# arcosoph/nanowakeword

Hardware: AMD Instinct MI355X
Metric: clips/sec (1 s @16 kHz PCM->logits) (higher is better)
Workload: dtype f32; 1 GPU; cnn head on (101,64) log-mel, batch=4096/GPU, 1 s 16 kHz mono int16 clips, 64-mel 25 ms/10 ms center frontend, fused STFT+mel HIP kernel, fp32; clips_per_gpu=4096, n_samples=16000, parallelism=batch-split x1

## Files before the change

### nanowakeword_amd/csrc/layers.h

```cpp
#pragma once
#include <hip/hip_runtime.h>

#include <map>
#include <mutex>
#include <utility>
inline hipError_t nww_allow_lds(const void* func, size_t bytes) {
    if (bytes <= 64 * 1024) return hipSuccess;
    static std::mutex mu;
    static std::map<std::pair<int, const void*>, size_t> done;
    int dev = 0;
    hipError_t e = hipGetDevice(&dev);
    if (e != hipSuccess) return e;
    std::lock_guard<std::mutex> lk(mu);
    size_t& cur = done[std::make_pair(dev, func)];
    if (bytes > cur) {
        e = hipFuncSetAttribute(func, hipFuncAttributeMaxDynamicSharedMemorySize, (int)bytes);
        if (e != hipSuccess) return e;
        cur = bytes;
    }
    return hipSuccess;
}

__device__ __forceinline__ float nww_silu(float v) {
    return v * __builtin_amdgcn_rcpf(1.0f + __builtin_amdgcn_exp2f(v * -1.4426950408889634f));
// ... 31 lines not shown
    int h2 = 0; float a_scale = 1.0f, c_scale = 1.0f, a_clamp = 0.0f;
    int a_blocked = 0;
    const float* A2 = nullptr; int lda2 = 0; const float* W2 = nullptr; int K2 = 0;
    const float* alpha2 = nullptr; const float* beta2 = nullptr;
};
size_t gemm_x3_weight_bytes(int N, int K);
hipError_t launch_split_weights_x3(const float* W, void* out, int N, int K, hipStream_t s);
hipError_t launch_split_weights_h2(const float* W, void* out, int N, int K, float scale, hipStream_t s);
bool gemm_x3_usable(const GemmArgs& g);
bool gemm_writes_partials(const GemmArgs& g);
hipError_t launch_gemm_x3(const GemmArgs& g, hipStream_t s);
int gemm_recommended_splitk(long long M, int N, int K, int cu_count);
hipError_t launch_gemm(const GemmArgs& g, hipStream_t s);

struct Conv3Args {
    const float* in; const float* w; const float* bias; const float* alpha; const float* beta;
    float* out; int B, Cin, Cout, H, W; int act; int pool;
    int nhwc_out = 0;
};
hipError_t launch_conv3x3(const Conv3Args& a, hipStream_t s);

hipError_t launch_dwconv3x3_nhwc(const float* in, const float* wt, float* d_out, float* xs_out, int B, int C, int H,
                                 int W, int sh, int sw, hipStream_t s, int act16 = 0, float out_mul = 1.0f);
hipError_t launch_layernorm_parts(const float* parts, int nparts, size_t part_stride, const float* in_bias, float* y, const float* w,
                                  const float* b, int R, int D, int act, hipStream_t s);
hipError_t launch_layernorm(const float* x, float* y, const float* w, const float* b, int R, int D, int act,
                            hipStream_t s);
hipError_t launch_mean_mid(const float* in, float* out, int B, int L, int D, hipStream_t s, int act16 = 0, float unscale = 1.0f);
hipError_t launch_ln_mean(const float* x, float* out, const float* w, const float* b, int B, int L, int D, hipStream_t s);
hipError_t launch_avgpool(const float* in, float* out, int BC, int H, int W, int kh, int kw, int sh, int sw, int oh,
                          int ow, hipStream_t s);
hipError_t launch_unary(const float* x, float* y, size_t n, int act, hipStream_t s);
hipError_t launch_scale_add_pe(float* x, const float* pe, int B, int T, int D, float scale, hipStream_t s);
hipError_t launch_glu(const float* in, float* out, int R, int D, hipStream_t s);
hipError_t launch_dwconv1d_bn_swish(const float* x, const float* w , const float* bias, const float* alpha,
                                    const float* beta, float* y, int B, int T, int D, int K, hipStream_t s);
hipError_t launch_mha_core(const float* qkv, float* out, int B, int T, int D, int n_head, hipStream_t s);
bool mha_mfma_supported(int T, int D, int n_head);
hipError_t launch_mha_mfma(const float* qkv, float* out, int B, int T, int D, int n_head, int cus, hipStream_t s, int head_major = 0);
bool mha_head_dim_supported(int head_dim);
bool mha_h2_supported(int T, int D, int n_head);
hipError_t launch_mha_h2(const float* qkv, float* out, int B, int T, int D, int n_head, int cus, hipStream_t s, int head_major = 0, int exact_sub = 0);
hipError_t launch_crnn_seq(const float* in, float* out, int B, int C, int H, int W, hipStream_t s);
struct GruArgs {
    const float* xg; const float* w_hh; const float* b_hh;
    float* seq_out; int ld_seq; float* last_out; int ld_last; int col_off;
    int B, T, H, reverse, steps;
    int products = 0;
    float w_scale = 1.0f;
    const float* xg2 = nullptr; size_t xg2_bstride = 0; const float* b_hh2 = nullptr; int col_off2 = 0;
    int ldw = 0;
    const float* x_in = nullptr; const float* w_ih = nullptr; const float* b_ih = nullptr;
    int fin = 0; float x_scale = 1.0f, x_clamp = 0.0f, wi_scale = 1.0f;
    const void* w_packed = nullptr;
    int cu_count = 256;
    int dbg = 0;
};
size_t rnn_wide_weight_bytes(int gates, int H);
hipError_t launch_rnn_pad_weights(const float* w_hh, float* out, int gates, int H, hipStream_t s);
hipError_t launch_gru(const GruArgs& a, hipStream_t s);
hipError_t launch_transpose3x3(const float* w, float* out, int nfilters, hipStream_t s);
hipError_t launch_transpose_planes(const float* in, float* out, int B, int R, int C, hipStream_t s);
bool rnn_x3_usable(const GruArgs& a);
hipError_t launch_rnn_x3(const GruArgs& a, int gates, hipStream_t s);
bool rnn_stream_usable(const GruArgs& a);
size_t rnn_stream_packed_bytes(int gates, int H);
hipError_t launch_rnn_stream_pack(const float* w_hh, void* packed, int gates, int H, float w_scale, hipStream_t s);
hipError_t launch_rnn_stream(const GruArgs& a, int gates, hipStream_t s);
hipError_t launch_lstm(const GruArgs& a, hipStream_t s);

struct TailArgs {
    const float* x; int Kin;
    const float *We, *be; int E;
    const float *W0, *b0, *w3, *b3;
    float *emb, *logits, *probs;
    int B, act;
    const float* parts = nullptr; int nparts = 0; size_t part_stride = 0;
    const float *in_bias = nullptr, *in_alpha = nullptr, *in_beta = nullptr; int in_act = 0;
    unsigned int* done_flag = nullptr; unsigned int done_seq = 0;
    const float *ln0_w = nullptr, *ln0_b = nullptr;
    int n_mid = 0;
    const float *mid_W[4] = {nullptr, nullptr, nullptr, nullptr}, *mid_b[4] = {nullptr, nullptr, nullptr, nullptr};
    const float *mid_lnw[4] = {nullptr, nullptr, nullptr, nullptr}, *mid_lnb[4] = {nullptr, nullptr, nullptr, nullptr};
};
bool tail_supported(int Kin, int E);
hipError_t launch_classifier_tail(const TailArgs& a, hipStream_t s);
```

### nanowakeword_amd/csrc/layers.hip

```cpp
#include <hip/hip_runtime.h>
#include <stdint.h>
#include <stdlib.h>
#include "layers.h"
#include "split_h2.h"

typedef float f32x16 __attribute__((ext_vector_type(16)));
typedef float f32x4 __attribute__((ext_vector_type(4)));

__device__ __forceinline__ float act_apply(float v, int act) {
    switch (act) {
        case ACT_RELU: return fmaxf(v, 0.0f);
        case ACT_GELU: return nww_gelu(v);
        case ACT_SILU: return v / (1.0f + expf(-v));
        case ACT_SIGMOID: return 1.0f / (1.0f + expf(-v));
        default: return v;
    }
}

template <int ACT>
__device__ __forceinline__ float act_ct(float v) {
    if (ACT == ACT_RELU) return fmaxf(v, 0.0f);
    if (ACT == ACT_GELU) return nww_gelu(v);
    if (ACT == ACT_SILU) return v / (1.0f + expf(-v));
    if (ACT == ACT_SIGMOID) return 1.0f / (1.0f + expf(-v));
// ... 1607 lines not shown
                    const size_t o = (size_t)(b0 + cc) * Kin + k;
                    float acc = 0.0f;
                    for (int z0 = 0; z0 < a.nparts; z0 += 8) {
                        float pv[8];
#pragma unroll
                        for (int j = 0; j < 8; ++j) pv[j] = z0 + j < a.nparts ? a.parts[(size_t)(z0 + j) * a.part_stride + o] : 0.0f;
#pragma unroll
                        for (int j = 0; j < 8; ++j)
                            if (z0 + j < a.nparts) acc = (z0 + j == 0) ? pv[j] : acc + pv[j];
                    }
                    v = acc + (a.in_bias ? a.in_bias[k] : 0.0f);
                    if (a.in_alpha) v = v * a.in_alpha[k] + a.in_beta[k];
                    v = act_apply(v, a.in_act);
                } else {
                    v = a.x[(size_t)(b0 + cc) * Kin + k];
                }
            }
            xs[cc * ldx + k] = v;
        }
        __syncthreads();
        if (a.ln0_w) {
            tile_ln(xs, xs, a.ln0_w, a.ln0_b);
            __syncthreads();
            for (int m = 0; m < a.n_mid; ++m) {
                const float* Wm = a.mid_W[m];
                const bool vm = (Kin & 3) == 0 && ((reinterpret_cast<uintptr_t>(Wm) & 15) == 0);
                for (int e0 = g; e0 < Kin; e0 += 4 * NG) {
                    const int e1 = min(e0 + NG, Kin - 1), e2 = min(e0 + 2 * NG, Kin - 1), e3 = min(e0 + 3 * NG, Kin - 1);
                    float acc[4];
                    tail_dot4(xs + c * ldx, Wm + (size_t)e0 * Kin, Wm + (size_t)e1 * Kin, Wm + (size_t)e2 * Kin, Wm + (size_t)e3 * Kin, Kin, vm, acc);
                    const int eo[4] = {e0, e0 + NG, e0 + 2 * NG, e0 + 3 * NG};
#pragma unroll
                    for (int r = 0; r < 4; ++r)
                        if (eo[r] < Kin) ys[c * ldx + eo[r]] = acc[r] + a.mid_b[m][eo[r]];
                }
                __syncthreads();
                tile_ln(ys, xs, a.mid_lnw[m], a.mid_lnb[m]);
                __syncthreads();
            }
        }
        for (int e0 = g; e0 < E; e0 += 4 * NG) {
            const int e1 = min(e0 + NG, E - 1), e2 = min(e0 + 2 * NG, E - 1), e3 = min(e0 + 3 * NG, E - 1);
            float acc[4];
            tail_dot4(xs + c * ldx, a.We + (size_t)e0 * Kin, a.We + (size_t)e1 * Kin, a.We + (size_t)e2 * Kin, a.We + (size_t)e3 * Kin, Kin, vx, acc);
            const int es_[4] = {e0, e0 + NG, e0 + 2 * NG, e0 + 3 * NG};
#pragma unroll
            for (int r = 0; r < 4; ++r)
                if (es_[r] < E) {
                    const float v = acc[r] + (a.be ? a.be[es_[r]] : 0.0f);
                    es[c * lde + es_[r]] = v;
                    if (b0 + c < a.B) a.emb[(size_t)(b0 + c) * E + es_[r]] = v;
                }
        }
        __syncthreads();
        for (int j0 = g; j0 < Hd; j0 += 4 * NG) {
            const int j1 = min(j0 + NG, Hd - 1), j2 = min(j0 + 2 * NG, Hd - 1), j3 = min(j0 + 3 * NG, Hd - 1);
            float acc[4];
            tail_dot4(es + c * lde, a.W0 + (size_t)j0 * E, a.W0 + (size_t)j1 * E, a.W0 + (size_t)j2 * E, a.W0 + (size_t)j3 * E, E, ve, acc);
            const int js[4] = {j0, j0 + NG, j0 + 2 * NG, j0 + 3 * NG};
#pragma unroll
            for (int r = 0; r < 4; ++r)
                if (js[r] < Hd) hs[c * ldh + js[r]] = act_ct<ACT>(acc[r] + a.b0[js[r]]);
        }
        __syncthreads();
        if (tid < CT && b0 + tid < a.B) {
            const float* hr = hs + tid * ldh;
            float acc = 0.0f;
            for (int j = 0; j < Hd; ++j) acc = fmaf(hr[j], a.w3[j], acc);
            const float l = acc + a.b3[0];
            a.logits[b0 + tid] = l;
            if (a.probs) a.probs[b0 + tid] = 1.0f / (1.0f + expf(-l));
            if (a.done_flag) __threadfence_system();
        }
        __syncthreads();
    }
    if (a.done_flag && gridDim.x == 1 && tid == 0) {
        __threadfence_system();
        __hip_atomic_store(a.done_flag, a.done_seq, __ATOMIC_RELEASE, __HIP_MEMORY_SCOPE_SYSTEM);
    }
}

bool tail_supported(int Kin, int E) { return Kin >= 1 && Kin <= 512 && E >= 2 && E <= 256 && (E % 2) == 0; }

hipError_t launch_classifier_tail(const TailArgs& a, hipStream_t s) {
    if (!tail_supported(a.Kin, a.E)) return hipErrorInvalidValue;
    if (a.ln0_w && (a.Kin > 256 || a.n_mid < 0 || a.n_mid > 4)) return hipErrorInvalidValue;
    const size_t lds = (size_t)16 * ((a.ln0_w ? 2 : 1) * (((a.Kin + 3) & ~3) + 4) + (((a.E + 3) & ~3) + 4) + (a.E / 2 + 1)) * sizeof(float);
    static const int ct4_max = 1024;
    const bool small = a.B <= 4 || (a.B > 16 && a.B <= ct4_max);
    const int ct = small ? 4 : 16;
    int grid = (a.B + ct - 1) / ct;
    if (grid > 1024) grid = 1024;
    if (grid < 1) grid = 1;
    if (small) {
#define TAIL_CALL(A) hipLaunchKernelGGL((classifier_tail_kernel<A, 4>), dim3(grid), dim3(256), lds, s, a)
        NWW_DISPATCH_ACT(a.act, TAIL_CALL)
#undef TAIL_CALL
    } else {
#define TAIL_CALL(A) hipLaunchKernelGGL((classifier_tail_kernel<A, 16>), dim3(grid), dim3(256), lds, s, a)
        NWW_DISPATCH_ACT(a.act, TAIL_CALL)
#undef TAIL_CALL
    }
    return hipGetLastError();
}
```

### nanowakeword_amd/csrc/nww_plan.hip

```cpp
#include "nww_internal.h"
#include "bc_chain.h"

const Knobs& nww_knobs() {
    static const Knobs k = [] {
        auto env = [](const char* name, int d) { const char* e = getenv(name); return e ? atoi(e) : d; };
        Knobs r;
        r.trunk = env("NWW_TRUNK", 1); r.conv_mfma = env("NWW_CONV_MFMA", 1); r.conv3_x3 = env("NWW_CONV3_X3", 1);
        r.gemm_x3 = env("NWW_GEMM_X3", 1); r.lin_x3 = env("NWW_LIN_X3", 1); r.ffn_fused = env("NWW_FFN_FUSED", 1);
        r.attn_fused = env("NWW_ATTN_FUSED", 1); r.mha_mfma = env("NWW_MHA_MFMA", 1); r.bc_front = env("NWW_BC_FRONT", 1);
        r.bc_chain = env("NWW_BC_CHAIN", 1); r.tail = env("NWW_TAIL", 1); r.stream_inc = env("NWW_STREAM_INC", 3);
        r.f16_range_log2 = env("NWW_F16_RANGE_LOG2", 16);
        return r;
    }();
    return k;
}

namespace {
using Shape = std::vector<int64_t>;
struct SpecBuilder {
    std::vector<std::string>& keys;
    std::map<std::string, HostTensor>& t;
    void add(const std::string& k, Shape s) { keys.push_back(k); t[k].shape = std::move(s); }
    void lin(const std::string& p, int out, int in) { add(p + ".weight", {out, in}); add(p + ".bias", {out}); }
    void ln(const std::string& p, int d) { add(p + ".weight", {d}); add(p + ".bias", {d}); }
// ... 139 lines not shown
    const float* W(const std::string& k) const {
        auto it = h->tensors.find(k);
        return it == h->tensors.end() || !it->second.loaded ? nullptr : h->d_weights + it->second.dev_off;
    }
    void need(int buf, size_t floats_per_clip) {
        if (h->buf_per_clip[buf] < floats_per_clip) h->buf_per_clip[buf] = floats_per_clip;
    }
    void add(const std::string& name, std::function<hipError_t(Run&)> fn) { h->plan.push_back({name, std::move(fn)}); }
    void pop_last() { if (!h->plan.empty()) h->plan.pop_back(); }
    std::string tail_name; int tail_in = 99, tail_K = 0; const float *tail_W = nullptr, *tail_b = nullptr;
    struct DnnBody { bool on = false; const float *ln0_w = nullptr, *ln0_b = nullptr; int n_mid = 0; const float* mid[4][4] = {}; } dnn;
};

std::vector<float> f16_fetch(nww_handle* h, const float* d, size_t n) {
    std::vector<float> v(n, 0.0f);
    if (d && n) {
        (void)hipStreamSynchronize(h->own_stream);
        if (hipMemcpy(v.data(), d, n * sizeof(float), hipMemcpyDeviceToHost) != hipSuccess) v.assign(n, INFINITY);
    }
    return v;
}
double f16_pow2_floor(double x) { int e; (void)std::frexp(x, &e); return std::ldexp(1.0, e - 1); }
float f16_scale(double bound) {
    if (!(bound > 1e-30)) bound = 1e-30;
    if (!(bound < 1e30)) return 0.0f;
    double s = f16_pow2_floor(65504.0 / (bound * 1.02));
    if (s > 1099511627776.0) s = 1099511627776.0;
    return (float)s;
}
float f16_wscale(const std::vector<float>& w) {
    double m = 0;
    for (float x : w) m = std::fmax(m, std::fabs((double)x));
    return f16_scale(m * 2.0);
}
double f16_layer_bound(const std::vector<float>& w, int Cout, int K, const std::vector<float>& b, bool has_b,
                       const std::vector<float>& al, const std::vector<float>& be, bool has_bn, double in_bound) {
    double worst = 0;
    for (int c = 0; c < Cout; ++c) {
        double t = 0;
        for (int k = 0; k < K; ++k) t += std::fabs((double)w[(size_t)c * K + k]);
        t = t * in_bound + (has_b ? std::fabs((double)b[c]) : 0.0);
        if (has_bn) t = t * std::fabs((double)al[c]) + std::fabs((double)be[c]);
        worst = std::fmax(worst, t);
    }
    return worst;
}
double f16_ln_bound(nww_handle* h, const float* w, const float* b, int D) {
    const auto hw = f16_fetch(h, w, D), hb = f16_fetch(h, b, D);
    double bound = 0.0;
    for (int k = 0; k < D; ++k) bound = std::fmax(bound, std::sqrt((double)D) * std::fabs((double)hw[k]) + std::fabs((double)hb[k]));
    return bound;
}
float f16_mean_scale(double bound) {
    const float s = bound < 1e30 ? (float)f16_pow2_floor(68719476736.0 / std::fmax(bound, 1e-30)) : 0.0f;
    return s > 0.0f && std::isfinite(s) ? s : 0.0f;
}

inline double f16_range_factor() {
    return std::ldexp(1.0, nww_knobs().f16_range_log2);
}
struct F16Range {
    double bound = 0.0, typ = 0.0;
    bool ok() const { return bound > 0.0 && typ > 0.0 && bound <= typ * f16_range_factor(); }
};
const F16Range F16_FEATURES{NWW_F16_FEATURE_BOUND, 32.0};
double f16_layer_typ(const std::vector<float>& w, int Cout, int K, const std::vector<float>& al, bool has_bn, double typ_in) {
    double acc = 0;
    for (int c = 0; c < Cout; ++c) {
        double q = 0;
        for (int k = 0; k < K; ++k) q += (double)w[(size_t)c * K + k] * (double)w[(size_t)c * K + k];
        acc += std::sqrt(q) * (has_bn ? std::fabs((double)al[c]) : 1.0);
    }
    return acc / (Cout > 0 ? Cout : 1) * typ_in;
}

inline const float* src(Run& r, int id) { return id == -1 ? r.x : id == -2 ? r.emb : id == -3 ? r.hid : r.buf[id]; }
inline float* dst(Run& r, int id) { return id == -2 ? r.emb : id == -3 ? r.hid : id == -4 ? r.logits : r.buf[id]; }

void add_gemm(PlanCtx& p, const std::string& name, int in_id, int out_id, int rows_per_clip, int N, int K,
              const float* W, const float* bias, int act, const float* alpha = nullptr, const float* beta = nullptr,
              int res_id = 99, float rscale = 1.f, bool* a_blocked_inout = nullptr, bool feeds_tail = false, bool feeds_ln = false,
              F16Range a_range = F16Range{}, bool a_bound_assumed = false) {
    const double a_bound = a_range.ok() ? a_range.bound : 0.0;
    if (out_id >= 0) p.need(out_id, (size_t)rows_per_clip * N);
    const int x3_mode = nww_knobs().gemm_x3;
    const bool small_square = N <= 160 && K > 64 && K <= 160;
    const bool use_x3 = p.h->conv_products != 0 &&
                        (x3_mode == 2 ? (N >= 32 && K >= 32)
                         : x3_mode == 3 ? (K >= 4096 && N >= 64 && N <= 256)
                         : (x3_mode == 1 && N >= 64 && K >= 32 && !small_square));
    const void* wx3 = nullptr;
    float h2_as = 0.0f, h2_ws = 0.0f;
    if (use_x3 && p.h->f16 && a_bound > 0.0) {
        h2_as = f16_scale(a_bound);
        if (h2_as > 0.0f) h2_ws = f16_wscale(f16_fetch(p.h, W, (size_t)N * K));
    }
    const bool h2_req = h2_as > 0.0f && h2_ws > 0.0f;
    if (use_x3) {
        const X3Key key{W, h2_req ? 1 : 0, h2_req ? h2_ws : 0.0f};
        auto it = p.h->x3_weights.find(key);
        if (it == p.h->x3_weights.end()) {
            void* d = nullptr;
            if (hipMalloc(&d, gemm_x3_weight_bytes(N, K)) == hipSuccess &&
                (h2_req ? launch_split_weights_h2(W, d, N, K, h2_ws, p.h->own_stream) : launch_split_weights_x3(W, d, N, K, p.h->own_stream)) == hipSuccess)
                it = p.h->x3_weights.emplace(key, d).first;
            else if (d) (void)hipFree(d);
        }
        if (it != p.h->x3_weights.end()) wx3 = it->second;
    }
    const bool h2 = h2_req && wx3 != nullptr;
    if (h2 && a_bound_assumed && in_id == -1) p.h->clamps_features = true;
    const int a_blocked = (a_blocked_inout && *a_blocked_inout && wx3 && K % 32 == 0 && rows_per_clip == 1) ? K / 32 : 0;
    if (a_blocked_inout) *a_blocked_inout = a_blocked != 0;
    if (K >= 2048 && (size_t)16 * rows_per_clip * N > p.h->splitk_per_clip) p.h->splitk_per_clip = (size_t)16 * rows_per_clip * N;
    p.add("gemm:" + name + (h2 && wx3 ? " [f16x3]" : ""), [=](Run& r) {
        GemmArgs g;
        g.A = src(r, in_id); g.lda = K; g.W = W; g.C = dst(r, out_id); g.ldc = N;
        g.M = r.B * rows_per_clip; g.N = N; g.K = K; g.bias = bias; g.alpha = alpha; g.beta = beta; g.act = act;
        g.res = res_id == 99 ? nullptr : src(r, res_id); g.ldres = N; g.rscale = rscale;
        g.Wx3 = wx3;
        if (h2) { g.h2 = 1; g.a_scale = h2_as; g.c_scale = 1.0f / (h2_as * h2_ws); g.a_clamp = a_bound_assumed ? (float)a_bound : 0.0f; }
        g.a_blocked = a_blocked;
        g.splitk = gemm_recommended_splitk(g.M, N, K, r.cu_count);
        if (wx3 && x3_mode != 2 && K >= 2048) { g.splitk = K >= 8192 ? K / 800 : K / 512; if (g.splitk > 16) g.splitk = 16; if (g.splitk < 1) g.splitk = 1; }
        g.splitk_ws = r.splitk_ws;
        if (g.splitk > 1 && (size_t)g.splitk * g.M * N > r.splitk_floats) g.splitk = 1;
        r.deferred.active = false;
        const bool partials = g.splitk > 1 && g.splitk_ws && gemm_writes_partials(g);
        if (feeds_tail && g.M <= 8 && partials && !g.res) {
            g.defer_reduce = true;
            r.deferred.active = true; r.deferred.out_id = out_id; r.deferred.parts = g.splitk; r.deferred.stride = (size_t)g.M * N;
            r.deferred.bias = bias; r.deferred.alpha = alpha; r.deferred.beta = beta; r.deferred.act = act;
        }
        if (feeds_ln && partials && !g.res && !alpha && act == ACT_NONE && N <= 256) {
            g.defer_reduce = true;
            r.deferred.active = true; r.deferred.out_id = out_id; r.deferred.parts = g.splitk; r.deferred.stride = (size_t)g.M * N;
            r.deferred.bias = bias; r.deferred.alpha = nullptr; r.deferred.beta = nullptr; r.deferred.act = ACT_NONE;
        }
        return launch_gemm(g, r.stream);
    });
}

bool add_lin_x3(PlanCtx& p, const std::string& name, int in_id, int out_id, int rows_per_clip, int N, int K, const float* W,
                const float* bias, int epi, int res_id = 99, float rscale = 1.f, const float* ln_w = nullptr,
                const float* ln_b = nullptr, int qkv_T = 0, int qkv_dh = 0, const float* res_tab = nullptr) {
    if (!nww_knobs().lin_x3 || p.h->conv_products != 6 || !lin_x3_supported(K, N, true)) return false;
    const int parts = epi == 2 ? 2 : 1;
    float ws = 0.0f;
    if (p.h->f16) ws = f16_wscale(f16_fetch(p.h, W, (size_t)parts * N * K));
    const bool h2 = ws > 0.0f;
    if (!lin_x3_supported(K, N, h2)) return false;
    const int terms = h2 ? 2 : 3;
    void* packed = nullptr;
    if (hipMalloc(&packed, lin_x3_packed_bytes(K, N, parts, terms)) != hipSuccess) return false;
    if (launch_lin_x3_pack(W, bias, packed, K, N, parts, N, p.h->own_stream, terms, h2 ? ws : 1.0f) != hipSuccess) { (void)hipFree(packed); return false; }
    p.h->packed_weights.push_back(packed);
    p.need(out_id, (size_t)rows_per_clip * N);
    const float w_un = h2 ? 1.0f / ws : 1.0f;
    p.add("lin_x3:" + name + (h2 ? " [f16x3]" : ""), [=](Run& r) {
        LinArgs a;
        a.x = src(r, in_id); a.ldx = K; a.out = dst(r, out_id); a.ldc = N;
        a.res = res_tab ? res_tab : res_id == 99 ? nullptr : src(r, res_id); a.ldres = N; a.rscale = rscale;
        a.ln_w = ln_w; a.ln_b = ln_b; a.packed = static_cast<const unsigned char*>(packed);
        a.M = r.B * rows_per_clip; a.N = N; a.qkv_T = qkv_T; a.qkv_dh = qkv_dh;
        a.h2 = h2 ? 1 : 0; a.w_un = w_un;
        return launch_lin_x3(a, K, epi, ln_w != nullptr, r.stream);
    });
    return true;
}

void add_linear(PlanCtx& p, const std::string& name, int in_id, int out_id, int rows_per_clip, int N, int K, const float* W,
                const float* bias, int res_id = 99, float rscale = 1.f) {
    if (!add_lin_x3(p, name, in_id, out_id, rows_per_clip, N, K, W, bias, res_id == 99 ? 0 : 1, res_id, rscale))
        add_gemm(p, name, in_id, out_id, rows_per_clip, N, K, W, bias, ACT_NONE, nullptr, nullptr, res_id, rscale);
}

void set_tail(PlanCtx& p, const std::string& name, int in_id, int K, const float* W, const float* b) {
    p.tail_name = name; p.tail_in = in_id; p.tail_K = K; p.tail_W = W; p.tail_b = b;
}

void add_conv(PlanCtx& p, const std::string& name, int in_id, int out_id, int Cin, int Cout, int H, int W,
              const float* w, const float* bias, const float* alpha, const float* beta, int act, int pool, int nhwc_out = 0) {
    const int Ho = pool ? H / 2 : H, Wo = pool ? W / 2 : W;
    p.need(out_id, (size_t)Cout * Ho * Wo);
    p.add("conv3x3:" + name, [=](Run& r) {
        Conv3Args a{src(r, in_id), w, bias, alpha, beta, dst(r, out_id), r.B, Cin, Cout, H, W, act, pool};
        a.nhwc_out = nhwc_out;
        return launch_conv3x3(a, r.stream);
    });
}

static int trunk_fits(int C1, int H, int W) { int per_cu = 0; return trunk_pick_strips(C1, H, W, &per_cu); }
bool add_trunk(PlanCtx& p, const std::string& name, int in_id, int out_id, int C1, int C2, int H, int W,
               const float* w1, const float* b1, const float* al1, const float* be1, const float* w2,
               const float* b2, const float* al2, const float* be2, int act, const bool* out_blocked = nullptr,
               F16Range in_range = F16Range{}, F16Range* out_range = nullptr) {
    if (out_range) *out_range = F16Range{};
    const double in_bound = in_range.ok() ? in_range.bound : 0.0;
    if (!nww_knobs().trunk || C1 != 16 || C2 != 32 || H < 4 || W < 4 || trunk_fits(C1, H, W) == 0) return false;
    p.need(out_id, (size_t)C2 * (H / 4) * (W / 4));
    const int max_grid = p.h->cu_count;
    const int x3 = p.h->conv_products;
    if ((x3 == 6 || x3 == 9) && trunk_b_pick_strips(H, W) > 0) {
        void* packed = nullptr;
        if (hipMalloc(&packed, trunk_b_packed_bytes()) != hipSuccess) return false;
        float f_in = 0.0f, f_s1 = 0.0f, f_w1 = 0.0f, f_w2 = 0.0f;
        double bound2 = 0.0, typ2 = 0.0;
        if (p.h->f16 && x3 == 6 && in_bound > 0.0 && (act == ACT_RELU || act == ACT_GELU || act == ACT_SILU)) {
            const auto hw1 = f16_fetch(p.h, w1, (size_t)C1 * 9), hw2 = f16_fetch(p.h, w2, (size_t)C2 * C1 * 9);
            const auto hb1 = f16_fetch(p.h, b1, C1), hb2 = f16_fetch(p.h, b2, C2);
            const auto ha1 = f16_fetch(p.h, al1, C1), he1 = f16_fetch(p.h, be1, C1), ha2 = f16_fetch(p.h, al2, C2), he2 = f16_fetch(p.h, be2, C2);
            const double bound1 = f16_layer_bound(hw1, C1, 9, hb1, b1 != nullptr, ha1, he1, al1 != nullptr, in_bound);
// ... 970 lines not shown
    set_tail(p, "output_proj", t1, D, p.W("model.output_proj.weight"), p.W("model.output_proj.bias"));
    return NWW_OK;
}

int plan_tcn(PlanCtx& p) {
    const nww_config& c = p.h->cfg;
    const int T = c.in_rows, F = c.in_cols;
    const int k = c.layer_dim, nl = c.n_crnn_channels;
    const int* ch = c.crnn_channels;
    const int last = 5;
    p.need(last, (size_t)ch[nl - 1]);
    auto key = [](int i, const char* part) { return "model.tcn_blocks." + std::to_string(i) + "." + part; };
    bool fused = false;
    if (p.h->f16 && p.h->conv_products == 6) {
        TcnArgs a;
        a.T = T; a.F = F; a.L = nl; a.k = k;
        for (int i = 0; i < nl; ++i) a.ch[i] = ch[i];
        std::vector<void*> packs;
        bool ok = tcn_x3_plan(a);
        int cin = F;
        for (int i = 0; ok && i < nl; ++i) {
            auto pack = [&](const char* part, int ci, int taps, TcnConv& cv) {
                const float* w = p.W(key(i, (std::string(part) + ".weight").c_str()));
                const float ws = f16_wscale(f16_fetch(p.h, w, (size_t)ch[i] * ci * taps));
                void* d = nullptr;
                if (!(ws > 0.0f) || hipMalloc(&d, tcn_x3_packed_bytes(ci, ch[i], taps)) != hipSuccess) return false;
                packs.push_back(d);
                if (launch_tcn_x3_pack(w, d, ci, ch[i], taps, ws, p.h->own_stream) != hipSuccess) return false;
                cv.packed = static_cast<const unsigned char*>(d);
                cv.bias = p.W(key(i, (std::string(part) + ".bias").c_str()));
                cv.w_un = 1.0f / ws;
                return true;
            };
            ok = pack("conv1", cin, k, a.c1[i]) && pack("conv2", ch[i], k, a.c2[i]) && (cin == ch[i] || pack("downsample", cin, 1, a.ds[i]));
            cin = ch[i];
        }
        if (ok) {
            for (void* d : packs) p.h->packed_weights.push_back(d);
            p.add("tcn_x3:" + std::to_string(nl) + " blocks, last " + std::to_string(a.S) + " steps of " + std::to_string(T) + " [f16x3]",
                  [=](Run& r) {
                      TcnArgs g = a;
                      g.x = r.x; g.out = r.buf[last]; g.B = r.B;
                      return launch_tcn_x3(g, r.stream);
                  });
            fused = true;
        } else {
            for (void* d : packs) (void)hipFree(d);
        }
    }
    if (!fused) {
        const int col = 0, hid = 1, rsd = 4;
        int in = -1, cin = F;
        for (int i = 0; i < nl; ++i) {
            const int co = ch[i], dil = 1 << i, out = i % 2 == 0 ? 2 : 3;
            const std::string q = "model.tcn_blocks." + std::to_string(i);
            p.need(col, (size_t)T * k * (cin > co ? cin : co));
            p.add("im2col:" + q + ".conv1", [=](Run& r) { return launch_tcn_im2col(src(r, in), r.buf[col], r.B, T, cin, k, dil, r.stream); });
            add_gemm(p, q + ".conv1+relu", col, hid, T, co, cin * k, p.W(key(i, "conv1.weight")), p.W(key(i, "conv1.bias")), ACT_RELU);
            p.add("im2col:" + q + ".conv2", [=](Run& r) { return launch_tcn_im2col(r.buf[hid], r.buf[col], r.B, T, co, k, dil, r.stream); });
            int res = in;
            if (cin != co) {
                add_gemm(p, q + ".downsample", in, rsd, T, co, cin, p.W(key(i, "downsample.weight")), p.W(key(i, "downsample.bias")), ACT_NONE);
                res = rsd;
            }
            add_gemm(p, q + ".conv2+relu+res", col, out, T, co, co * k, p.W(key(i, "conv2.weight")), p.W(key(i, "conv2.bias")), ACT_RELU,
                     nullptr, nullptr, res, 1.0f);
            p.add("unary:relu " + q, [=](Run& r) { return launch_unary(r.buf[out], r.buf[out], (size_t)r.B * T * co, ACT_RELU, r.stream); });
            in = out; cin = co;
        }
        const int fin = in, C = cin;
        p.add("last_row:tcn_out[:, :, T - 1]", [=](Run& r) { return launch_tcn_last_row(r.buf[fin], r.buf[last], r.B, T, C, r.stream); });
    }
    set_tail(p, "fc", last, ch[nl - 1], p.W("model.fc.weight"), p.W("model.fc.bias"));
    return NWW_OK;
}

void plan_tail(PlanCtx& p) {
    const int E = p.h->cfg.embedding_dim, act = p.h->cfg.activation;
    if (nww_knobs().tail && tail_supported(p.tail_K, E)) {
        const float *We = p.tail_W, *be = p.tail_b, *W0 = p.W("classifier.0.weight"), *b0 = p.W("classifier.0.bias"),
                    *w3 = p.W("classifier.3.weight"), *b3 = p.W("classifier.3.bias");
        const int tin = p.tail_in, tK = p.tail_K;
        const PlanCtx::DnnBody dnn = p.dnn;
        p.add("tail:" + p.tail_name + "+classifier", [=](Run& r) {
            TailArgs t{src(r, tin), tK, We, be, E, W0, b0, w3, b3, r.emb, r.logits, r.probs, r.B, act};
            if (dnn.on) {
                t.ln0_w = dnn.ln0_w; t.ln0_b = dnn.ln0_b; t.n_mid = dnn.n_mid;
                for (int i = 0; i < dnn.n_mid; ++i) { t.mid_W[i] = dnn.mid[i][0]; t.mid_b[i] = dnn.mid[i][1]; t.mid_lnw[i] = dnn.mid[i][2]; t.mid_lnb[i] = dnn.mid[i][3]; }
            }
            if (r.deferred.active && r.deferred.out_id == tin) {
                t.parts = r.splitk_ws; t.nparts = r.deferred.parts; t.part_stride = r.deferred.stride;
                t.in_bias = r.deferred.bias; t.in_alpha = r.deferred.alpha; t.in_beta = r.deferred.beta; t.in_act = r.deferred.act;
            }
            r.deferred.active = false;
            r.need_sigmoid = false;
            if (r.done_flag && r.B <= 16) { t.done_flag = r.done_flag; t.done_seq = r.done_seq; r.done_armed = true; }
            return launch_classifier_tail(t, r.stream);
        });
    } else {
        add_gemm(p, p.tail_name, p.tail_in, -2, 1, E, p.tail_K, p.tail_W, p.tail_b, ACT_NONE);
        add_gemm(p, "classifier.0", -2, -3, 1, E / 2, E, p.W("classifier.0.weight"), p.W("classifier.0.bias"), act);
        add_gemm(p, "classifier.3", -3, -4, 1, 1, E / 2, p.W("classifier.3.weight"), p.W("classifier.3.bias"), ACT_NONE);
    }
}

}

extern "C" int nww_finalize(nww_handle* h) {
    if (!h) return NWW_ERR_INVALID;
    if (h->finalized) return NWW_OK;
    HIP_TRY(h, hipSetDevice(h->cfg.device));
    for (const auto& k : h->keys)
        if (!h->tensors[k].loaded) return fail(h, NWW_ERR_MISSING, "Missing key(s) in state_dict: '%s'", k.c_str());
    fold_batchnorms(h);
    if (h->cfg.head_type == NWW_HEAD_BCRESNET) transpose_depthwise(h);
    int rc = upload_weight_arena(h);
    if (rc == NWW_OK) rc = build_frontend_tables(h);
    if (rc != NWW_OK) return rc;
    PlanCtx p{h};
    switch (h->cfg.head_type) {
        case NWW_HEAD_DNN: rc = plan_dnn(p); break;
        case NWW_HEAD_CNN: rc = plan_cnn(p); break;
        case NWW_HEAD_E2E_DNN: rc = plan_e2e_dnn(p); break;
        case NWW_HEAD_CRNN: rc = plan_crnn(p); break;
        case NWW_HEAD_GRU: rc = plan_gru(p); break;
        case NWW_HEAD_BCRESNET: rc = plan_bcresnet(p); break;
        case NWW_HEAD_CONFORMER: rc = plan_conformer(p); break;
        case NWW_HEAD_TRANSFORMER: rc = plan_transformer(p); break;
        case NWW_HEAD_TCN: rc = plan_tcn(p); break;
    }
    if (rc != NWW_OK) return rc;
    plan_tail(p);
    HIP_TRY(h, hipStreamSynchronize(h->own_stream));
    if (!h->plan_error.empty()) return fail(h, NWW_ERR_HIP, "%s", h->plan_error.c_str());
    h->finalized = true;
    return NWW_OK;
}
```

Before: 9.050 million clips/s.

## Add persistent LDS-resident-weight classifier tail kernel for large batches

Adds a persistent classifier-tail kernel for batches above 1024. It loads the embedding and classifier weights into LDS once per workgroup, then loops over 8-clip tiles and prefetches the next tile's inputs from global memory. It also allows the preceding split-K GEMM to defer its reduction into this kernel at large batch sizes, which removes a separate reduce pass. The cost is high LDS use per workgroup, which limits occupancy to at most 2 workgroups per CU, plus extra code paths with their own alignment checks.

```diff
diff --git a/nanowakeword_amd/csrc/layers.h b/nanowakeword_amd/csrc/layers.h
--- a/nanowakeword_amd/csrc/layers.h
+++ b/nanowakeword_amd/csrc/layers.h
@@ -137,6 +137,8 @@
     int n_mid = 0;
     const float *mid_W[4] = {nullptr, nullptr, nullptr, nullptr}, *mid_b[4] = {nullptr, nullptr, nullptr, nullptr};
     const float *mid_lnw[4] = {nullptr, nullptr, nullptr, nullptr}, *mid_lnb[4] = {nullptr, nullptr, nullptr, nullptr};
+    int cu_count = 256;
 };
 bool tail_supported(int Kin, int E);
+bool tail_batch_runs(int B, int Kin, int E, bool dnn_body, int nparts);
 hipError_t launch_classifier_tail(const TailArgs& a, hipStream_t s);
diff --git a/nanowakeword_amd/csrc/layers.hip b/nanowakeword_amd/csrc/layers.hip
--- a/nanowakeword_amd/csrc/layers.hip
+++ b/nanowakeword_amd/csrc/layers.hip
@@ -1713,11 +1713,187 @@
 
 bool tail_supported(int Kin, int E) { return Kin >= 1 && Kin <= 512 && E >= 2 && E <= 256 && (E % 2) == 0; }
 
+constexpr int TB_CT = 8, TB_NG = 256 / TB_CT;
+constexpr int TAIL_CT4_MAX = 1024;
+constexpr size_t TB_LDS_MAX = 96 * 1024;
+constexpr int TB_WG_PER_CU = 2;
+
+__host__ __device__ inline int tb_pitch(int n) { const int p = ((n + 3) & ~3) + 4; return ((p >> 2) & 1) ? p : p + 4; }
+static size_t tb_lds_bytes(int Kin, int E) {
+    const int Hd = E / 2, h4 = (Hd + 3) & ~3;
+    return sizeof(float) * ((size_t)(E + TB_CT) * tb_pitch(Kin) + (size_t)(Hd + TB_CT) * tb_pitch(E) + E + 2 * h4 + TB_CT * (Hd + 1));
+}
+
+bool tail_batch_runs(int B, int Kin, int E, bool dnn_body, int nparts) {
+    return B > TAIL_CT4_MAX && !dnn_body && tail_supported(Kin, E) && (Kin % 4) == 0 && (E % 4) == 0 &&
+           (nparts == 0 || (nparts <= 16 && Kin <= 128)) &&
+           tb_lds_bytes(Kin, E) <= TB_LDS_MAX;
+}
+
+template <int NB>
+__device__ __forceinline__ void tb_load(const float* __restrict__ src, int i0, int n4, f32x4 (&v)[NB]) {
+#pragma unroll
+    for (int j = 0; j < NB; ++j) v[j] = reinterpret_cast<const f32x4*>(src)[min(i0 + 256 * j, n4 - 1)];
+}
+template <int NB>
+__device__ __forceinline__ void tb_store(float* dstp, int i0, int n4, int K4, int pitch, const f32x4 (&v)[NB]) {
+#pragma unroll
+    for (int j = 0; j < NB; ++j) {
+        const int i = min(i0 + 256 * j, n4 - 1), r = i / K4;
+        *reinterpret_cast<f32x4*>(dstp + r * pitch + 4 * (i - r * K4)) = v[j];
+    }
+}
+
+template <int R, class F>
+__device__ __forceinline__ void tb_layer(const float* xr, const float* Ws, int pW, int N, int K, int g, F&& out) {
+    for (int e0 = g; e0 < N; e0 += R * TB_NG) {
+        const float* wr[R];
+        float acc[R];
+#pragma unroll
+        for (int r = 0; r < R; ++r) { wr[r] = Ws + min(e0 + r * TB_NG, N - 1) * pW; acc[r] = 0.0f; }
+#pragma unroll 4
+        for (int k = 0; k < K; k += 4) {
+            const float4 x = *reinterpret_cast<const float4*>(xr + k);
+#pragma unroll
+            for (int r = 0; r < R; ++r) {
+                const float4 w = *reinterpret_cast<const float4*>(wr[r] + k);
+                acc[r] = fmaf(x.x, w.x, acc[r]); acc[r] = fmaf(x.y, w.y, acc[r]); acc[r] = fmaf(x.z, w.z, acc[r]); acc[r] = fmaf(x.w, w.w, acc[r]);
+            }
+        }
+#pragma unroll
+        for (int r = 0; r < R; ++r)
+            if (e0 + r * TB_NG < N) out(e0 + r * TB_NG, acc[r]);
+    }
+}
+template <class F>
+__device__ __forceinline__ void tb_layer_any(const float* xr, const float* Ws, int pW, int N, int K, int g, F&& out) {
+    const int per = (N + TB_NG - 1) / TB_NG;
+    if (per >= 3) tb_layer<4>(xr, Ws, pW, N, K, g, out);
+    else if (per == 2) tb_layer<2>(xr, Ws, pW, N, K, g, out);
+    else tb_layer<1>(xr, Ws, pW, N, K, g, out);
+}
+
+template <int ACT, bool PARTS>
+__global__ void __launch_bounds__(256) __attribute__((amdgpu_waves_per_eu(1, 2))) classifier_tail_batch_kernel(TailArgs a) {
+    constexpr int CT = TB_CT, NPF = PARTS ? 16 : 4;
+    extern __shared__ __attribute__((aligned(16))) float tsm[];
+    const int Kin = a.Kin, E = a.E, Hd = E / 2, K4 = Kin / 4, E4 = E / 4;
+    const int pK = tb_pitch(Kin), pE = tb_pitch(E), ldh = Hd + 1, h4 = (Hd + 3) & ~3;
+    float* Wes = tsm;
+    float* W0s = Wes + E * pK;
+    float* xs = W0s + Hd * pE;
+    float* es = xs + CT * pK;
+    float* bes = es + CT * pE;
+    float* b0s = bes + E;
+    float* w3s = b0s + h4;
+    float* hs = w3s + h4;
+    const int tid = threadIdx.x, n4 = CT * K4;
+    const int B = a.B, step = gridDim.x * CT;
+    int pc[PARTS ? 1 : 4], pq[PARTS ? 1 : 4];
+#pragma unroll
+    for (int j = 0; j < (PARTS ? 1 : 4); ++j) { const int i = min(tid + 256 * j, n4 - 1); pc[j] = i / K4; pq[j] = i - pc[j] * K4; }
+    f32x4 pf[NPF];
+    auto request = [&](int b0) {
+        if (PARTS) {
+            const size_t o = (size_t)min(b0 + pc[0], B - 1) * Kin + 4 * pq[0];
+#pragma unroll
+            for (int z = 0; z < 16; ++z) pf[z] = *reinterpret_cast<const f32x4*>(a.parts + (size_t)min(z, a.nparts - 1) * a.part_stride + o);
+        } else {
+#pragma unroll
+            for (int j = 0; j < 4; ++j) pf[j] = *reinterpret_cast<const f32x4*>(a.x + (size_t)min(b0 + pc[j], B - 1) * Kin + 4 * pq[j]);
+        }
+    };
+    int b0 = blockIdx.x * CT;
+    const float bev = a.be ? a.be[min(tid, E - 1)] : 0.0f, b0v = a.b0[min(tid, Hd - 1)], w3v = a.w3[min(tid, Hd - 1)], b3 = a.b3[0];
+    float ib[4] = {0.f, 0.f, 0.f, 0.f}, ia[4] = {0.f, 0.f, 0.f, 0.f}, ie[4] = {0.f, 0.f, 0.f, 0.f};
+    if (PARTS) {
+        const float *pb = a.in_bias ? a.in_bias : a.parts, *pa = a.in_alpha ? a.in_alpha : a.parts, *pe = a.in_alpha ? a.in_beta : a.parts;
+#pragma unroll
+        for (int i = 0; i < 4; ++i) { const int k = 4 * pq[0] + i; ib[i] = pb[k]; ia[i] = pa[k]; ie[i] = pe[k]; }
+    }
+    request(b0);
+    {
+        f32x4 wv[8], uv[4];
+        tb_load(a.We, tid, E * K4, wv);
+        tb_load(a.W0, tid, Hd * E4, uv);
+        asm volatile("" : "+v"(wv[0]), "+v"(wv[1]), "+v"(wv[2]), "+v"(wv[3]), "+v"(wv[4]), "+v"(wv[5]), "+v"(wv[6]), "+v"(wv[7]),
+                          "+v"(uv[0]), "+v"(uv[1]), "+v"(uv[2]), "+v"(uv[3]), "+v"(pf[0]), "+v"(pf[NPF - 1]));
+        tb_store(Wes, tid, E * K4, K4, pK, wv);
+        tb_store(W0s, tid, Hd * E4, E4, pE, uv);
+        for (int i0 = tid + 8 * 256; i0 < E * K4; i0 += 8 * 256) { f32x4 v[8]; tb_load(a.We, i0, E * K4, v); tb_store(Wes, i0, E * K4, K4, pK, v); }
+        for (int i0 = tid + 4 * 256; i0 < Hd * E4; i0 += 4 * 256) { f32x4 v[4]; tb_load(a.W0, i0, Hd * E4, v); tb_store(W0s, i0, Hd * E4, E4, pE, v); }
+    }
+    if (tid < E) bes[tid] = bev;
+    if (tid < Hd) { b0s[tid] = b0v; w3s[tid] = w3v; }
+    for (; b0 < B; b0 += step) {
+        int t = threadIdx.x;
+        asm volatile("" : "+v"(t));
+        const int c = t % CT, g = t / CT;
+        if (PARTS) {
+            float v[4] = {pf[0].x, pf[0].y, pf[0].z, pf[0].w};
+#pragma unroll
+            for (int z = 1; z < 16; ++z)
+                if (z < a.nparts) { v[0] += pf[z].x; v[1] += pf[z].y; v[2] += pf[z].z; v[3] += pf[z].w; }
+#pragma unroll
+            for (int i = 0; i < 4; ++i) {
+                float u = v[i] + (a.in_bias ? ib[i] : 0.0f);
+                if (a.in_alpha) u = u * ia[i] + ie[i];
+                v[i] = act_apply(u, a.in_act);
+                if (b0 + pc[0] >= B) v[i] = 0.0f;
+            }
+            if (t < n4) *reinterpret_cast<f32x4*>(xs + pc[0] * pK + 4 * pq[0]) = f32x4{v[0], v[1], v[2], v[3]};
+        } else {
+#pragma unroll
+            for (int j = 0; j < 4; ++j)
+                if (t + 256 * j < n4) *reinterpret_cast<f32x4*>(xs + pc[j] * pK + 4 * pq[j]) = b0 + pc[j] < B ? pf[j] : f32x4{0.f, 0.f, 0.f, 0.f};
+        }
+        if (b0 + step < B) request(b0 + step);
+        __syncthreads();
+        tb_layer_any(xs + c * pK, Wes, pK, E, Kin, g, [&](int e, float acc) { es[c * pE + e] = acc + bes[e]; });
+        __syncthreads();
+        for (int i = t; i < CT * E4; i += 256) {
+            const int cc = i / E4, q = i - cc * E4;
+            if (b0 + cc < B) *reinterpret_cast<float4*>(a.emb + (size_t)(b0 + cc) * E + 4 * q) = *reinterpret_cast<const float4*>(es + cc * pE + 4 * q);
+        }
+        tb_layer_any(es + c * pE, W0s, pE, Hd, E, g, [&](int j, float acc) { hs[c * ldh + j] = act_ct<ACT>(acc + b0s[j]); });
+        __syncthreads();
+        if (t < CT && b0 + t < B) {
+            const float* hr = hs + t * ldh;
+            float acc = 0.0f;
+            for (int j = 0; j < Hd; ++j) acc = fmaf(hr[j], w3s[j], acc);
+            const float l = acc + b3;
+            a.logits[b0 + t] = l;
+            if (a.probs) a.probs[b0 + t] = 1.0f / (1.0f + expf(-l));
+        }
+    }
+}
+
+static bool aligned16(const void* p) { return (reinterpret_cast<uintptr_t>(p) & 15) == 0; }
+
 hipError_t launch_classifier_tail(const TailArgs& a, hipStream_t s) {
     if (!tail_supported(a.Kin, a.E)) return hipErrorInvalidValue;
     if (a.ln0_w && (a.Kin > 256 || a.n_mid < 0 || a.n_mid > 4)) return hipErrorInvalidValue;
+    if (tail_batch_runs(a.B, a.Kin, a.E, a.ln0_w != nullptr, a.parts ? a.nparts : 0) && !a.done_flag && (!a.parts || a.nparts >= 1) && aligned16(a.We) && aligned16(a.W0) &&
+        aligned16(a.emb) && aligned16(a.parts ? a.parts : a.x) && (a.part_stride % 4) == 0) {
+        const size_t lds = tb_lds_bytes(a.Kin, a.E);
+        int grid = (a.B + TB_CT - 1) / TB_CT;
+        const int wgs = (int)std::min<size_t>(TB_WG_PER_CU, (160 * 1024) / lds);
+        if (grid > a.cu_count * wgs) grid = a.cu_count * wgs;
+#define TAILB_CALL(A)                                                                                                       \
+    {                                                                                                                       \
+        const void* f = a.parts ? reinterpret_cast<const void*>(classifier_tail_batch_kernel<A, true>)                      \
+                                : reinterpret_cast<const void*>(classifier_tail_batch_kernel<A, false>);                    \
+        const hipError_t ea = nww_allow_lds(f, lds);                                                                        \
+        if (ea != hipSuccess) return ea;                                                                                    \
+        if (a.parts) hipLaunchKernelGGL((classifier_tail_batch_kernel<A, true>), dim3(grid), dim3(256), lds, s, a);         \
+        else hipLaunchKernelGGL((classifier_tail_batch_kernel<A, false>), dim3(grid), dim3(256), lds, s, a);                \
+    }
+        NWW_DISPATCH_ACT(a.act, TAILB_CALL)
+#undef TAILB_CALL
+        return hipGetLastError();
+    }
     const size_t lds = (size_t)16 * ((a.ln0_w ? 2 : 1) * (((a.Kin + 3) & ~3) + 4) + (((a.E + 3) & ~3) + 4) + (a.E / 2 + 1)) * sizeof(float);
-    static const int ct4_max = 1024;
+    static const int ct4_max = TAIL_CT4_MAX;
     const bool small = a.B <= 4 || (a.B > 16 && a.B <= ct4_max);
     const int ct = small ? 4 : 16;
     int grid = (a.B + ct - 1) / ct;
diff --git a/nanowakeword_amd/csrc/nww_plan.hip b/nanowakeword_amd/csrc/nww_plan.hip
--- a/nanowakeword_amd/csrc/nww_plan.hip
+++ b/nanowakeword_amd/csrc/nww_plan.hip
@@ -245,6 +245,7 @@
               int res_id = 99, float rscale = 1.f, bool* a_blocked_inout = nullptr, bool feeds_tail = false, bool feeds_ln = false,
               F16Range a_range = F16Range{}, bool a_bound_assumed = false) {
     const double a_bound = a_range.ok() ? a_range.bound : 0.0;
+    const int tail_E = p.h->cfg.embedding_dim;
     if (out_id >= 0) p.need(out_id, (size_t)rows_per_clip * N);
     const int x3_mode = nww_knobs().gemm_x3;
     const bool small_square = N <= 160 && K > 64 && K <= 160;
@@ -290,7 +291,7 @@
         if (g.splitk > 1 && (size_t)g.splitk * g.M * N > r.splitk_floats) g.splitk = 1;
         r.deferred.active = false;
         const bool partials = g.splitk > 1 && g.splitk_ws && gemm_writes_partials(g);
-        if (feeds_tail && g.M <= 8 && partials && !g.res) {
+        if (feeds_tail && partials && !g.res && (g.M <= 8 || tail_batch_runs(g.M, N, tail_E, false, g.splitk))) {
             g.defer_reduce = true;
             r.deferred.active = true; r.deferred.out_id = out_id; r.deferred.parts = g.splitk; r.deferred.stride = (size_t)g.M * N;
             r.deferred.bias = bias; r.deferred.alpha = alpha; r.deferred.beta = beta; r.deferred.act = act;
@@ -1427,8 +1428,10 @@
                     *w3 = p.W("classifier.3.weight"), *b3 = p.W("classifier.3.bias");
         const int tin = p.tail_in, tK = p.tail_K;
         const PlanCtx::DnnBody dnn = p.dnn;
-        p.add("tail:" + p.tail_name + "+classifier", [=](Run& r) {
+        const bool batch_kernel = tail_batch_runs(1 << 20, tK, E, dnn.on, 0);
+        p.add("tail:" + p.tail_name + "+classifier" + (batch_kernel ? " (large batches: persistent, weights in LDS)" : ""), [=](Run& r) {
             TailArgs t{src(r, tin), tK, We, be, E, W0, b0, w3, b3, r.emb, r.logits, r.probs, r.B, act};
+            t.cu_count = r.cu_count;
             if (dnn.on) {
                 t.ln0_w = dnn.ln0_w; t.ln0_b = dnn.ln0_b; t.n_mid = dnn.n_mid;
                 for (int i = 0; i < dnn.n_mid; ++i) { t.mid_W[i] = dnn.mid[i][0]; t.mid_b[i] = dnn.mid[i][1]; t.mid_lnw[i] = dnn.mid[i][2]; t.mid_lnb[i] = dnn.mid[i][3]; }
```

New measurement: 9.198 million clips/s, median of 6. +1.6%, better.
